# theblackcat102/edgedict

Hardware: NVIDIA H100
Metric: audio-sec/sec E6D2 B=32 T=1000 U=128 V=1024 training step (higher is better)
Workload: dtype bf16

## Files before the change

### edgedict_b200/csrc/elementwise.cu

```cuda
#include "common.cuh"
#include "../../include/edgedict_b200.h"

namespace {

constexpr int LN_WARPS = 8;

template <int PL>
__global__ void __launch_bounds__(LN_WARPS * 32)
layernorm_fwd_kernel(const float* __restrict__ x, const float* __restrict__ res,
                     const float* __restrict__ gamma, const float* __restrict__ beta,
                     float* __restrict__ y, __nv_bfloat16* __restrict__ y16,
                     float* __restrict__ mean, float* __restrict__ rstd, long rows, int H, float eps) {
    const int lane = threadIdx.x & 31;
    const long wstride = (long)gridDim.x * LN_WARPS;
    for (long r = (long)blockIdx.x * LN_WARPS + (threadIdx.x >> 5); r < rows; r += wstride) {
        const float* xr = x + r * H;
        const float* rr = res ? res + r * H : nullptr;
        float v[PL];
        float s = 0.f;
#pragma unroll
        for (int i = 0; i < PL; ++i) {
            int c = lane + i * 32;
            v[i] = 0.f;
            if (c < H) {
                float t = xr[c];
                if (rr) t += rr[c];
                v[i] = t;
                s += t;
            }
        }
        const float mu = warp_sum(s) / H;
        float q = 0.f;
#pragma unroll
        for (int i = 0; i < PL; ++i) {
            int c = lane + i * 32;
            if (c < H) { float d = v[i] - mu; q += d * d; }
        }
        const float rs = rsqrtf(warp_sum(q) / H + eps);
        if (lane == 0) {
            if (mean) mean[r] = mu;
            if (rstd) rstd[r] = rs;
        }
#pragma unroll
        for (int i = 0; i < PL; ++i) {
            int c = lane + i * 32;
            if (c < H) {
                float o = (v[i] - mu) * rs * gamma[c] + beta[c];
                y[r * H + c] = o;
                if (y16) y16[r * H + c] = __float2bfloat16(o);
            }
        }
    }
}

template <int PL>
__global__ void __launch_bounds__(LN_WARPS * 32)
layernorm_bwd_kernel(const float* __restrict__ dy, const float* __restrict__ x,
                     const float* __restrict__ res, const float* __restrict__ gamma,
                     const float* __restrict__ mean, const float* __restrict__ rstd,
                     float* __restrict__ dz, long rows, int H) {
    const int lane = threadIdx.x & 31, w = threadIdx.x >> 5;
    const long wstride = (long)gridDim.x * LN_WARPS;
    for (long r = (long)blockIdx.x * LN_WARPS + w; r < rows; r += wstride) {
        const float mu = mean[r], rs = rstd[r];
        float xh[PL], g[PL];
        float s1 = 0.f, s2 = 0.f;
#pragma unroll
        for (int i = 0; i < PL; ++i) {
            int c = lane + i * 32;
            xh[i] = 0.f; g[i] = 0.f;
            if (c < H) {
                float z = x[r * H + c];
                if (res) z += res[r * H + c];
                xh[i] = (z - mu) * rs;
                g[i] = dy[r * H + c] * gamma[c];
                s1 += g[i];
                s2 += g[i] * xh[i];
            }
        }
        s1 = warp_sum(s1) / H;
        s2 = warp_sum(s2) / H;
#pragma unroll
        for (int i = 0; i < PL; ++i) {
            int c = lane + i * 32;
            if (c < H) dz[r * H + c] = rs * (g[i] - s1 - xh[i] * s2);
        }
    }
}

constexpr int LNB_WARPS = 4;
template <int NV>
__global__ void __launch_bounds__(LNB_WARPS * 32)
layernorm_bwd_fused_kernel(const float* __restrict__ dy, const float* __restrict__ x, const float* __restrict__ res,
                           const float* __restrict__ gamma, const float* __restrict__ mean,
                           const float* __restrict__ rstd, float* __restrict__ dz, long rows, int H) {
    const int lane = threadIdx.x & 31, w = threadIdx.x >> 5;
    const int H4 = H >> 2;
    const long wstride = (long)gridDim.x * LNB_WARPS;
    const float inv_h = 1.f / (float)H;
    const float4* g4 = reinterpret_cast<const float4*>(gamma);
    for (long r = (long)blockIdx.x * LNB_WARPS + w; r < rows; r += wstride) {
        const float mu = mean[r], rs = rstd[r];
        const float4* dy4 = reinterpret_cast<const float4*>(dy + r * H);
        const float4* x4 = reinterpret_cast<const float4*>(x + r * H);
        const float4* r4 = res ? reinterpret_cast<const float4*>(res + r * H) : nullptr;
        float4 d[NV], xh[NV];
        float s1 = 0.f, s2 = 0.f;
#pragma unroll
        for (int i = 0; i < NV; ++i) {
            const int c = lane + i * 32;
            d[i] = make_float4(0.f, 0.f, 0.f, 0.f); xh[i] = d[i];
            if (c < H4) {
                d[i] = dy4[c];
                float4 z = x4[c];
                if (r4) { const float4 q = r4[c]; z.x += q.x; z.y += q.y; z.z += q.z; z.w += q.w; }
                xh[i] = make_float4((z.x - mu) * rs, (z.y - mu) * rs, (z.z - mu) * rs, (z.w - mu) * rs);
                const float4 gm = __ldg(g4 + c);
                const float4 g = make_float4(d[i].x * gm.x, d[i].y * gm.y, d[i].z * gm.z, d[i].w * gm.w);
                s1 += (g.x + g.y) + (g.z + g.w);
                s2 += (g.x * xh[i].x + g.y * xh[i].y) + (g.z * xh[i].z + g.w * xh[i].w);
            }
        }
        s1 = warp_sum(s1) * inv_h;
        s2 = warp_sum(s2) * inv_h;
        float4* dz4 = reinterpret_cast<float4*>(dz + r * H);
#pragma unroll
        for (int i = 0; i < NV; ++i) {
            const int c = lane + i * 32;
            if (c < H4) {
                const float4 gm = __ldg(g4 + c);
                dz4[c] = make_float4(rs * (d[i].x * gm.x - s1 - xh[i].x * s2), rs * (d[i].y * gm.y - s1 - xh[i].y * s2),
                                     rs * (d[i].z * gm.z - s1 - xh[i].z * s2), rs * (d[i].w * gm.w - s1 - xh[i].w * s2));
            }
        }
    }
}

__global__ void __launch_bounds__(1024) layernorm_param_grad_kernel(const float* __restrict__ dy, const float* __restrict__ x,
                                                                     const float* __restrict__ res,
                                                                     const float* __restrict__ mean,
                                                                     const float* __restrict__ rstd, float* __restrict__ dgamma,
                                                                     float* __restrict__ dbeta, long rows, int H) {
    __shared__ float sg[128][9], sb[128][9];
    const int cx = threadIdx.x & 7, k = threadIdx.x >> 3;
    const int c = blockIdx.x * 8 + cx;
    float ag = 0.f, ab = 0.f;
    if (c < H) {
        for (long r = k; r < rows; r += 128) {
            float z = x[r * H + c];
            if (res) z += res[r * H + c];
            const float d = dy[r * H + c];
            ag += d * (z - mean[r]) * rstd[r];
            ab += d;
        }
    }
    sg[k][cx] = ag;
    sb[k][cx] = ab;
    __syncthreads();
#pragma unroll 1
    for (int st = 64; st > 0; st >>= 1) {
        if (k < st) { sg[k][cx] += sg[k + st][cx]; sb[k][cx] += sb[k + st][cx]; }
        __syncthreads();
    }
    if (k == 0 && c < H) {
        dgamma[c] += sg[0][cx];
        dbeta[c] += sb[0][cx];
    }
}

__global__ void time_reduce_fwd_kernel(const float* __restrict__ x, float* __restrict__ y,
                                       __nv_bfloat16* __restrict__ y16, int B, int T, int H) {
    const int T2 = (T + 1) / 2;
    const long n = (long)B * T2 * H;
    for (long i = (long)blockIdx.x * blockDim.x + threadIdx.x; i < n; i += (long)gridDim.x * blockDim.x) {
        int c = (int)(i % H);
        long bt = i / H;
        int t2 = (int)(bt % T2);
        int b = (int)(bt / T2);
        float a = x[((long)b * T + 2 * t2) * H + c];
        float bb = (2 * t2 + 1 < T) ? x[((long)b * T + 2 * t2 + 1) * H + c] : 0.f;
        float o = (a + bb) * 0.5f;
        y[i] = o;
        if (y16) y16[i] = __float2bfloat16(o);
    }
}
__global__ void time_reduce_bwd_kernel(const float* __restrict__ dy, float* __restrict__ dx, int B,
                                       int T, int H) {
    const int T2 = (T + 1) / 2;
    const long n = (long)B * T * H;
    for (long i = (long)blockIdx.x * blockDim.x + threadIdx.x; i < n; i += (long)gridDim.x * blockDim.x) {
        int c = (int)(i % H);
        long bt = i / H;
        int t = (int)(bt % T);
        int b = (int)(bt / T);
        dx[i] = 0.5f * dy[((long)b * T2 + t / 2) * H + c];
    }
}

template <typename I>
__global__ void embedding_fwd_kernel(const I* __restrict__ ids, const float* __restrict__ W,
                                     float* __restrict__ out, __nv_bfloat16* __restrict__ out16,
                                     int B, int U, int E, int prepend, int bos) {
    const int U1 = U + prepend;
    const long n = (long)B * U1 * E;
    for (long i = (long)blockIdx.x * blockDim.x + threadIdx.x; i < n; i += (long)gridDim.x * blockDim.x) {
        int e = (int)(i % E);
        long bu = i / E;
        int u = (int)(bu % U1);
        int b = (int)(bu / U1);
        long id = (prepend && u == 0) ? bos : (long)ids[(long)b * U + u - prepend];
        float v = W[id * E + e];
        out[i] = v;
        if (out16) out16[i] = __float2bfloat16(v);
    }
}
template <typename I>
__device__ __forceinline__ long emb_id(const I* ids, long pos, int U, int U1, int prepend, int bos) {
    const long b = pos / U1;
    const int u = (int)(pos % U1);
    return (prepend && u == 0) ? bos : (long)ids[b * U + u - prepend];
}
template <typename I>
__global__ void embedding_bwd_kernel(const I* __restrict__ ids, const float* __restrict__ dout,
                                     float* __restrict__ dW, int B, int U, int E, int prepend,
                                     int bos, int pad) {
    const int U1 = U + prepend;
    const long n = (long)B * U1;
    const int lane = threadIdx.x & 31;
    for (long i = ((long)blockIdx.x * blockDim.x + threadIdx.x) >> 5; i < n; i += ((long)gridDim.x * blockDim.x) >> 5) {
        const long id = emb_id(ids, i, U, U1, prepend, bos);
        if (id == pad) continue;
        bool first = true;
        for (long j = lane; j < i && first; j += 32) first = emb_id(ids, j, U, U1, prepend, bos) != id;
        if (!__all_sync(0xffffffffu, first)) continue;
        for (int e = lane; e < E; e += 32) {
            float acc = 0.f;
            for (long j = i; j < n; ++j)
                if (emb_id(ids, j, U, U1, prepend, bos) == id) acc += dout[j * E + e];
            dW[id * E + e] += acc;
        }
    }
}

__device__ __forceinline__ float tanh_fast(float x) {
    float y;
    asm("tanh.approx.f32 %0, %1;" : "=f"(y) : "f"(x));
    return y;
}
__device__ __forceinline__ uint32_t pack_bf16(float a, float b) {
    __nv_bfloat162 v = __floats2bfloat162_rn(a, b);
    return *reinterpret_cast<uint32_t*>(&v);
}
__device__ __forceinline__ float2 unpack_bf16(uint32_t u) {
    return __bfloat1622float2(*reinterpret_cast<__nv_bfloat162*>(&u));
}

__global__ void joint_hidden_fwd_f32_kernel(const float* __restrict__ ep, const float* __restrict__ dp,
                                            float* __restrict__ hid, int T, int U, int J) {
    const long bt = blockIdx.x;
    const int b = (int)(bt / T);
    const float* e = ep + bt * J;
    const float* d = dp + (long)b * U * J;
    float* o = hid + bt * (long)U * J;
    for (int i = threadIdx.x; i < U * J; i += blockDim.x) o[i] = tanhf(e[i % J] + d[i]);
}

__global__ void joint_hidden_fwd_bf16_kernel(const float* __restrict__ ep, const float* __restrict__ dp,
                                             __nv_bfloat16* __restrict__ hid, int T, int U, int J) {
    const long bt = blockIdx.x;
    const int b = (int)(bt / T);
    const int J8 = J / 8;
    for (int q = threadIdx.x; q < J8; q += blockDim.x) {
        const float4 e0 = *reinterpret_cast<const float4*>(ep + bt * J + q * 8);
        const float4 e1 = *reinterpret_cast<const float4*>(ep + bt * J + q * 8 + 4);
        const float* d = dp + (long)b * U * J + q * 8;
        __nv_bfloat16* o = hid + bt * (long)U * J + q * 8;
#pragma unroll 4
        for (int u = 0; u < U; ++u) {
            const float4 d0 = *reinterpret_cast<const float4*>(d + (long)u * J);
            const float4 d1 = *reinterpret_cast<const float4*>(d + (long)u * J + 4);
            uint4 v;
            v.x = pack_bf16(tanh_fast(e0.x + d0.x), tanh_fast(e0.y + d0.y));
            v.y = pack_bf16(tanh_fast(e0.z + d0.z), tanh_fast(e0.w + d0.w));
            v.z = pack_bf16(tanh_fast(e1.x + d1.x), tanh_fast(e1.y + d1.y));
            v.w = pack_bf16(tanh_fast(e1.z + d1.z), tanh_fast(e1.w + d1.w));
            *reinterpret_cast<uint4*>(o + (long)u * J) = v;
        }
    }
}

__global__ void joint_hidden_bwd_t_f32_kernel(float* __restrict__ dh, const float* __restrict__ hid,
                                              float* __restrict__ dep, int T, int U, int J) {
    const long bt = blockIdx.x;
    float* g = dh + bt * (long)U * J;
    const float* h = hid + bt * (long)U * J;
    for (int j = threadIdx.x; j < J; j += blockDim.x) {
        float acc = 0.f;
        for (int u = 0; u < U; ++u) {
            float hv = h[(long)u * J + j];
            float pv = g[(long)u * J + j] * (1.f - hv * hv);
            g[(long)u * J + j] = pv;
            acc += pv;
        }
        dep[bt * J + j] = acc;
    }
}
__global__ void joint_hidden_bwd_t_bf16_kernel(__nv_bfloat16* __restrict__ dh, const __nv_bfloat16* __restrict__ hid,
                                               float* __restrict__ dep, int T, int U, int J) {
    const long bt = blockIdx.x;
    const int J8 = J / 8;
    for (int q = threadIdx.x; q < J8; q += blockDim.x) {
        __nv_bfloat16* g = dh + bt * (long)U * J + q * 8;
        const __nv_bfloat16* h = hid + bt * (long)U * J + q * 8;
        float acc[8] = {0.f, 0.f, 0.f, 0.f, 0.f, 0.f, 0.f, 0.f};
#pragma unroll 4
        for (int u = 0; u < U; ++u) {
            const uint4 hv = *reinterpret_cast<const uint4*>(h + (long)u * J);
            uint4 gv = *reinterpret_cast<const uint4*>(g + (long)u * J);
            const uint32_t hw[4] = {hv.x, hv.y, hv.z, hv.w};
            uint32_t gw[4] = {gv.x, gv.y, gv.z, gv.w};
#pragma unroll
            for (int i = 0; i < 4; ++i) {
                const float2 hf = unpack_bf16(hw[i]), gf = unpack_bf16(gw[i]);
                const float p0 = gf.x * (1.f - hf.x * hf.x), p1 = gf.y * (1.f - hf.y * hf.y);
                acc[2 * i] += p0;
                acc[2 * i + 1] += p1;
                gw[i] = pack_bf16(p0, p1);
            }
            *reinterpret_cast<uint4*>(g + (long)u * J) = make_uint4(gw[0], gw[1], gw[2], gw[3]);
        }
        float* o = dep + bt * J + q * 8;
        *reinterpret_cast<float4*>(o) = make_float4(acc[0], acc[1], acc[2], acc[3]);
        *reinterpret_cast<float4*>(o + 4) = make_float4(acc[4], acc[5], acc[6], acc[7]);
    }
}
__global__ void joint_dep_reduce_bf16_kernel(const __nv_bfloat16* __restrict__ dpre, float* __restrict__ dep, int U, int J) {
    const long bt = blockIdx.x;
    const int J8 = J / 8;
    for (int q = threadIdx.x; q < J8; q += blockDim.x) {
        const __nv_bfloat16* g = dpre + bt * (long)U * J + q * 8;
        float acc[8] = {0.f, 0.f, 0.f, 0.f, 0.f, 0.f, 0.f, 0.f};
#pragma unroll 8
        for (int u = 0; u < U; ++u) {
            const uint4 gv = *reinterpret_cast<const uint4*>(g + (long)u * J);
            const uint32_t gw[4] = {gv.x, gv.y, gv.z, gv.w};
#pragma unroll
            for (int i = 0; i < 4; ++i) {
                const float2 gf = unpack_bf16(gw[i]);
                acc[2 * i] += gf.x;
                acc[2 * i + 1] += gf.y;
            }
        }
        float* o = dep + bt * J + q * 8;
        *reinterpret_cast<float4*>(o) = make_float4(acc[0], acc[1], acc[2], acc[3]);
        *reinterpret_cast<float4*>(o + 4) = make_float4(acc[4], acc[5], acc[6], acc[7]);
    }
}
__global__ void joint_hidden_bwd_u_f32_kernel(const float* __restrict__ dpre, float* __restrict__ ddp, int T,
                                              int U, int J) {
    const int b = blockIdx.x / U, u = blockIdx.x % U;
    const float* g = dpre + ((long)b * T * U + u) * J;
    for (int j = threadIdx.x; j < J; j += blockDim.x) {
        float acc = 0.f;
        for (int t = 0; t < T; ++t) acc += g[(long)t * U * J + j];
        ddp[((long)b * U + u) * J + j] = acc;
    }
}
__global__ void joint_hidden_bwd_u_bf16_kernel(const __nv_bfloat16* __restrict__ dpre, float* __restrict__ ddp,
                                               int T, int U, int J) {
    const int b = blockIdx.x / U, u = blockIdx.x % U;
    const int t0 = 0, t1 = T;
    const int J8 = J / 8;
    for (int q = threadIdx.x; q < J8; q += blockDim.x) {
        const __nv_bfloat16* g = dpre + ((long)b * T * U + u) * J + q * 8;
        float acc[8] = {0.f, 0.f, 0.f, 0.f, 0.f, 0.f, 0.f, 0.f};
#pragma unroll 4
        for (int t = t0; t < t1; ++t) {
            const uint4 gv = *reinterpret_cast<const uint4*>(g + (long)t * U * J);
            const uint32_t gw[4] = {gv.x, gv.y, gv.z, gv.w};
#pragma unroll
            for (int i = 0; i < 4; ++i) {
                const float2 gf = unpack_bf16(gw[i]);
                acc[2 * i] += gf.x;
                acc[2 * i + 1] += gf.y;
            }
        }
        float* o = ddp + ((long)b * U + u) * J + q * 8;
        *reinterpret_cast<float4*>(o) = make_float4(acc[0], acc[1], acc[2], acc[3]);
        *reinterpret_cast<float4*>(o + 4) = make_float4(acc[4], acc[5], acc[6], acc[7]);
    }
}

template <int RL, int CW>
__device__ __forceinline__ float colsum_tree(float (*sh)[CW + 1], float v, int k, int cx) {
    sh[k][cx] = v;
    __syncthreads();
#pragma unroll 1
    for (int st = RL / 2; st > 0; st >>= 1) {
        if (k < st) sh[k][cx] += sh[k + st][cx];
        __syncthreads();
    }
    return sh[0][cx];
}
template <typename TI>
__global__ void __launch_bounds__(1024) colsum_kernel(const TI* __restrict__ x, float* __restrict__ out, long rows, int N) {
    __shared__ float sh[32][33];
    const int cx = threadIdx.x & 31, k = threadIdx.x >> 5;
    const int c = blockIdx.x * 32 + cx;
    float acc = 0.f;
    if (c < N)
        for (long r = k; r < rows; r += 32) acc += (float)x[r * N + c];
    const float t = colsum_tree<32, 32>(sh, acc, k, cx);
    if (k == 0 && c < N) out[c] += t;
}

__global__ void __launch_bounds__(1024) colsum_bf16_vec_kernel(const __nv_bfloat16* __restrict__ x, float* __restrict__ out,
                                                               long rows, int N) {
    __shared__ float sh[512][17];
    const int half = threadIdx.x & 1, k = threadIdx.x >> 1;
    const int c0 = blockIdx.x * 16 + half * 8;
    float acc[8] = {0.f, 0.f, 0.f, 0.f, 0.f, 0.f, 0.f, 0.f};
    if (c0 < N) {
        const __nv_bfloat16* p = x + (long)k * N + c0;
        const long step = 512L * N;
        long r = k;
        for (; r + 3 * 512 < rows; r += 4 * 512) {
            uint4 v[4];
#pragma unroll
            for (int q = 0; q < 4; ++q) v[q] = *reinterpret_cast<const uint4*>(p + q * step);
#pragma unroll
            for (int q = 0; q < 4; ++q) {
                const uint32_t w[4] = {v[q].x, v[q].y, v[q].z, v[q].w};
#pragma unroll
                for (int i = 0; i < 4; ++i) {
                    const float2 f = __bfloat1622float2(*reinterpret_cast<const __nv_bfloat162*>(&w[i]));
                    acc[2 * i] += f.x;
                    acc[2 * i + 1] += f.y;
                }
            }
            p += 4 * step;
        }
        for (; r < rows; r += 512, p += step) {
            const uint4 v = *reinterpret_cast<const uint4*>(p);
            const uint32_t w[4] = {v.x, v.y, v.z, v.w};
#pragma unroll
            for (int i = 0; i < 4; ++i) {
                const float2 f = __bfloat1622float2(*reinterpret_cast<const __nv_bfloat162*>(&w[i]));
                acc[2 * i] += f.x;
                acc[2 * i + 1] += f.y;
            }
        }
    }
#pragma unroll 1
    for (int i = 0; i < 8; ++i) {
        const float t = colsum_tree<512, 16>(sh, acc[i], k, half * 8 + i);
        if (k == 0 && c0 < N) out[c0 + i] += t;
        __syncthreads();
    }
}

__global__ void cast_bf16_kernel(const float* __restrict__ x, __nv_bfloat16* __restrict__ y, long n) {
    long i = ((long)blockIdx.x * blockDim.x + threadIdx.x) * 4;
    const long stride = (long)gridDim.x * blockDim.x * 4;
    for (; i + 3 < n; i += stride) {
        float4 v = *reinterpret_cast<const float4*>(x + i);
        __nv_bfloat162 a = __floats2bfloat162_rn(v.x, v.y), b = __floats2bfloat162_rn(v.z, v.w);
        uint2 q;
        q.x = *reinterpret_cast<uint32_t*>(&a);
        q.y = *reinterpret_cast<uint32_t*>(&b);
        *reinterpret_cast<uint2*>(y + i) = q;
    }
    if (i < n) for (long k = i; k < n && k < i + 4; ++k) y[k] = __float2bfloat16(x[k]);
}

template <typename TI>
__global__ void transpose_to_bf16_kernel(const TI* __restrict__ x, __nv_bfloat16* __restrict__ y,
                                         long rows, long cols) {
    __shared__ float tile[32][33];
    long c0 = (long)blockIdx.x * 32, r0 = (long)blockIdx.y * 32;
    for (int i = threadIdx.y; i < 32; i += blockDim.y) {
        long r = r0 + i, c = c0 + threadIdx.x;
        tile[i][threadIdx.x] = (r < rows && c < cols) ? (float)x[r * cols + c] : 0.f;
    }
    __syncthreads();
    for (int i = threadIdx.y; i < 32; i += blockDim.y) {
        long c = c0 + i, r = r0 + threadIdx.x;
        if (r < rows && c < cols) y[c * rows + r] = __float2bfloat16(tile[threadIdx.x][i]);
    }
}

__global__ void adam_kernel(float* __restrict__ p, const float* __restrict__ g, float* __restrict__ m,
                            float* __restrict__ v, long n, float lr, float b1, float b2, float eps,
                            float wd, float bc1, float bc2, float gscale) {
    for (long i = (long)blockIdx.x * blockDim.x + threadIdx.x; i < n; i += (long)gridDim.x * blockDim.x) {
        float gi = g[i] * gscale;
        if (wd != 0.f) gi += wd * p[i];
        float mi = b1 * m[i] + (1.f - b1) * gi;
        float vi = b2 * v[i] + (1.f - b2) * gi * gi;
        m[i] = mi;
        v[i] = vi;
        float denom = sqrtf(vi) / sqrtf(bc2) + eps;
        p[i] -= (lr / bc1) * (mi / denom);
    }
}

__global__ void adam_ex_kernel(float* __restrict__ p, const float* __restrict__ g, float* __restrict__ m,
                               float* __restrict__ v, long n, float lr, float b1, float b2, float eps, float wd,
                               float bc1, float bc2, float gscale, const float* __restrict__ sumsq, float max_norm,
                               int adamw) {
    float coef = gscale;
    if (sumsq) {
        const float norm = sqrtf(*sumsq) * fabsf(gscale);
        if (!isfinite(norm)) return;
        if (max_norm > 0.f) {
            const float c = max_norm / (norm + 1e-6f);
            if (c < 1.f) coef *= c;
        }
    }
    for (long i = (long)blockIdx.x * blockDim.x + threadIdx.x; i < n; i += (long)gridDim.x * blockDim.x) {
        float gi = g[i] * coef;
        const float pi = p[i];
        if (!adamw && wd != 0.f) gi += wd * pi;
        const float mi = b1 * m[i] + (1.f - b1) * gi;
        const float vi = b2 * v[i] + (1.f - b2) * gi * gi;
        m[i] = mi;
        v[i] = vi;
        if (adamw) p[i] = pi - (lr * sqrtf(bc2) / bc1) * (wd * pi + mi / (sqrtf(vi) + eps));
        else p[i] = pi - (lr / bc1) * (mi / (sqrtf(vi) / sqrtf(bc2) + eps));
    }
}

__global__ void sumsq_kernel(const float* __restrict__ x, long n, float* __restrict__ out) {
    __shared__ float sh[33];
    float acc = 0.f;
    for (long i = (long)blockIdx.x * blockDim.x + threadIdx.x; i < n; i += (long)gridDim.x * blockDim.x)
        acc += x[i] * x[i];
    acc = block_sum(acc, sh);
    if (threadIdx.x == 0) atomicAdd(out, acc);
}

inline int ew_grid(long n, int threads) {
    long b = (n + threads - 1) / threads;
    long cap = (long)eb_num_sms() * 32;
    return (int)(b < 1 ? 1 : (b < cap ? b : cap));
}

}

#define ST(s) reinterpret_cast<cudaStream_t>(s)

EB_API int eb_layernorm_fwd(const float* x, const float* res, const float* gamma, const float* beta,
                            float* y, void* y_bf16, float* mean, float* rstd, long rows, int H,
                            float eps, void* stream) {
    if (!x || !gamma || !beta || !y || rows <= 0 || H <= 0 || H > 2048) return EB_ERR_INVALID;
    long blocks = (rows + LN_WARPS - 1) / LN_WARPS;
    long cap = (long)eb_num_sms() * 8;
    int grid = (int)(blocks < cap ? blocks : cap);
#define LN_FWD(PL) layernorm_fwd_kernel<PL><<<grid, LN_WARPS * 32, 0, ST(stream)>>>( \
        x, res, gamma, beta, y, (__nv_bfloat16*)y_bf16, mean, rstd, rows, H, eps)
    if (H <= 256) LN_FWD(8); else if (H <= 512) LN_FWD(16); else if (H <= 1024) LN_FWD(32); else LN_FWD(64);
#undef LN_FWD
    EB_CHECK_LAUNCH();
    return EB_OK;
}

EB_API int eb_layernorm_bwd(const float* dy, const float* x, const float* res, const float* gamma,
                            const float* mean, const float* rstd, float* dz, float* dgamma,
                            float* dbeta, long rows, int H, void* stream) {
    if (!dy || !x || !gamma || !mean || !rstd || !dz || !dgamma || !dbeta || H > 2048)
        return EB_ERR_INVALID;
    const bool vec_ok = H % 128 == 0 && H <= 1024 && rows > 0 &&
                        ((reinterpret_cast<uintptr_t>(dy) | reinterpret_cast<uintptr_t>(x) | reinterpret_cast<uintptr_t>(dz) |
                          reinterpret_cast<uintptr_t>(gamma) | (res ? reinterpret_cast<uintptr_t>(res) : 0)) & 15) == 0;
    if (vec_ok) {
        long blocks_f = (rows + LNB_WARPS - 1) / LNB_WARPS;
        long cap_f = (long)eb_num_sms() * 3;
        const int grid_f = (int)(blocks_f < cap_f ? blocks_f : cap_f);
#define LN_BWDF(NV) layernorm_bwd_fused_kernel<NV><<<grid_f, LNB_WARPS * 32, 0, ST(stream)>>>( \
        dy, x, res, gamma, mean, rstd, dz, rows, H)
        if (H <= 128) LN_BWDF(1); else if (H <= 256) LN_BWDF(2); else if (H <= 512) LN_BWDF(4); else LN_BWDF(8);
#undef LN_BWDF
    } else {
        long blocks = (rows + LN_WARPS - 1) / LN_WARPS;
        long cap = (long)eb_num_sms() * 8;
        int grid = (int)(blocks < cap ? blocks : cap);
#define LN_BWD(PL) layernorm_bwd_kernel<PL><<<grid, LN_WARPS * 32, 0, ST(stream)>>>( \
        dy, x, res, gamma, mean, rstd, dz, rows, H)
        if (H <= 256) LN_BWD(8); else if (H <= 512) LN_BWD(16); else if (H <= 1024) LN_BWD(32); else LN_BWD(64);
#undef LN_BWD
    }
    EB_CHECK_LAUNCH();
    layernorm_param_grad_kernel<<<(H + 7) / 8, 1024, 0, ST(stream)>>>(dy, x, res, mean, rstd, dgamma, dbeta, rows, H);
    EB_CHECK_LAUNCH();
    return EB_OK;
}

EB_API int eb_time_reduce_fwd(const float* x, float* y, void* y_bf16, int B, int T, int H, void* stream) {
    long n = (long)B * ((T + 1) / 2) * H;
    time_reduce_fwd_kernel<<<ew_grid(n, 256), 256, 0, ST(stream)>>>(x, y, (__nv_bfloat16*)y_bf16, B, T, H);
    EB_CHECK_LAUNCH();
    return EB_OK;
}
EB_API int eb_time_reduce_bwd(const float* dy, float* dx, int B, int T, int H, void* stream) {
    long n = (long)B * T * H;
    time_reduce_bwd_kernel<<<ew_grid(n, 256), 256, 0, ST(stream)>>>(dy, dx, B, T, H);
    EB_CHECK_LAUNCH();
    return EB_OK;
}

EB_API int eb_embedding_fwd(const void* ids, int ids_are_int64, const float* W, float* out,
                            void* out_bf16, int B, int U, int E, int prepend_bos, int bos, void* stream) {
    long n = (long)B * (U + (prepend_bos ? 1 : 0)) * E;
    if (n <= 0) return EB_OK;
    if (ids_are_int64)
        embedding_fwd_kernel<long long><<<ew_grid(n, 256), 256, 0, ST(stream)>>>(
            (const long long*)ids, W, out, (__nv_bfloat16*)out_bf16, B, U, E, prepend_bos ? 1 : 0, bos);
    else
        embedding_fwd_kernel<int><<<ew_grid(n, 256), 256, 0, ST(stream)>>>(
            (const int*)ids, W, out, (__nv_bfloat16*)out_bf16, B, U, E, prepend_bos ? 1 : 0, bos);
    EB_CHECK_LAUNCH();
    return EB_OK;
}
EB_API int eb_embedding_bwd(const void* ids, int ids_are_int64, const float* dout, float* dW, int B,
                            int U, int E, int prepend_bos, int bos, int pad, void* stream) {
    const long npos = (long)B * (U + (prepend_bos ? 1 : 0));
    if (npos <= 0 || E <= 0) return EB_OK;
    const long n = npos * 32;
    if (ids_are_int64)
        embedding_bwd_kernel<long long><<<ew_grid(n, 256), 256, 0, ST(stream)>>>(
            (const long long*)ids, dout, dW, B, U, E, prepend_bos ? 1 : 0, bos, pad);
    else
        embedding_bwd_kernel<int><<<ew_grid(n, 256), 256, 0, ST(stream)>>>(
            (const int*)ids, dout, dW, B, U, E, prepend_bos ? 1 : 0, bos, pad);
    EB_CHECK_LAUNCH();
    return EB_OK;
}

EB_API int eb_joint_hidden_fwd(const float* ep, const float* dp, void* hidden, int hidden_bf16, int B,
                               int T, int U, int J, void* stream) {
    if (!ep || !dp || !hidden) return EB_ERR_INVALID;
    if (hidden_bf16) {
        if (J % 8) return EB_ERR_INVALID;
        joint_hidden_fwd_bf16_kernel<<<B * T, 96, 0, ST(stream)>>>(ep, dp, (__nv_bfloat16*)hidden, T, U, J);
    } else {
        joint_hidden_fwd_f32_kernel<<<B * T, 256, 0, ST(stream)>>>(ep, dp, (float*)hidden, T, U, J);
    }
    EB_CHECK_LAUNCH();
    return EB_OK;
}

EB_API int eb_joint_hidden_bwd(void* dhidden_inout, const void* hidden, int is_bf16, float* dep,
                               float* ddp, int B, int T, int U, int J, void* stream) {
    if (!dhidden_inout || !hidden || !dep || !ddp) return EB_ERR_INVALID;
    if (is_bf16) {
        if (J % 8) return EB_ERR_INVALID;
        joint_hidden_bwd_t_bf16_kernel<<<B * T, 96, 0, ST(stream)>>>(
            (__nv_bfloat16*)dhidden_inout, (const __nv_bfloat16*)hidden, dep, T, U, J);
        EB_CHECK_LAUNCH();
        joint_hidden_bwd_u_bf16_kernel<<<B * U, 96, 0, ST(stream)>>>((const __nv_bfloat16*)dhidden_inout, ddp, T, U, J);
    } else {
        joint_hidden_bwd_t_f32_kernel<<<B * T, 256, 0, ST(stream)>>>(
            (float*)dhidden_inout, (const float*)hidden, dep, T, U, J);
        EB_CHECK_LAUNCH();
        joint_hidden_bwd_u_f32_kernel<<<B * U, 256, 0, ST(stream)>>>((const float*)dhidden_inout, ddp, T, U, J);
    }
    EB_CHECK_LAUNCH();
    return EB_OK;
}

EB_API int eb_joint_dpre_reduce(const void* dpre16, float* dep, float* ddp, int B, int T, int U, int J, void* stream) {
    if (!dpre16 || !dep || !ddp || B <= 0 || T <= 0 || U <= 0 || J <= 0 || J % 8 ||
        (reinterpret_cast<uintptr_t>(dpre16) & 15) || (reinterpret_cast<uintptr_t>(dep) & 15))
        return EB_ERR_INVALID;
    joint_dep_reduce_bf16_kernel<<<B * T, 96, 0, ST(stream)>>>((const __nv_bfloat16*)dpre16, dep, U, J);
    EB_CHECK_LAUNCH();
    joint_hidden_bwd_u_bf16_kernel<<<B * U, 96, 0, ST(stream)>>>((const __nv_bfloat16*)dpre16, ddp, T, U, J);
    EB_CHECK_LAUNCH();
    return EB_OK;
}

EB_API int eb_colsum(const void* x, int x_bf16, float* out, long rows, int N, void* stream) {
    if (!x || !out || rows <= 0 || N <= 0) return EB_ERR_INVALID;
    if (x_bf16 && N % 8 == 0 && (reinterpret_cast<uintptr_t>(x) & 15) == 0)
        colsum_bf16_vec_kernel<<<(N + 15) / 16, 1024, 0, ST(stream)>>>((const __nv_bfloat16*)x, out, rows, N);
    else if (x_bf16)
        colsum_kernel<__nv_bfloat16><<<(N + 31) / 32, 1024, 0, ST(stream)>>>((const __nv_bfloat16*)x, out, rows, N);
    else
        colsum_kernel<float><<<(N + 31) / 32, 1024, 0, ST(stream)>>>((const float*)x, out, rows, N);
    EB_CHECK_LAUNCH();
    return EB_OK;
}

EB_API int eb_cast_bf16(const float* x, void* y, long n, void* stream) {
    if (n <= 0) return EB_OK;
    if ((reinterpret_cast<uintptr_t>(x) & 15) || (reinterpret_cast<uintptr_t>(y) & 7)) return EB_ERR_INVALID;
    cast_bf16_kernel<<<ew_grid((n + 3) / 4, 256), 256, 0, ST(stream)>>>(x, (__nv_bfloat16*)y, n);
    EB_CHECK_LAUNCH();
    return EB_OK;
}

EB_API int eb_transpose_to_bf16(const void* x, int x_bf16, void* y, long rows, long cols, void* stream) {
    dim3 grid((unsigned)((cols + 31) / 32), (unsigned)((rows + 31) / 32));
    if (x_bf16)
        transpose_to_bf16_kernel<__nv_bfloat16><<<grid, dim3(32, 8), 0, ST(stream)>>>(
            (const __nv_bfloat16*)x, (__nv_bfloat16*)y, rows, cols);
    else
        transpose_to_bf16_kernel<float><<<grid, dim3(32, 8), 0, ST(stream)>>>((const float*)x, (__nv_bfloat16*)y, rows, cols);
    EB_CHECK_LAUNCH();
    return EB_OK;
}

EB_API int eb_adam_step(float* p, const float* g, float* m, float* v, long n, float lr, float beta1,
                        float beta2, float eps, float weight_decay, int step, float grad_scale,
                        void* stream) {
    if (!p || !g || !m || !v || n <= 0 || step < 1) return EB_ERR_INVALID;
    float bc1 = 1.f - powf(beta1, (float)step), bc2 = 1.f - powf(beta2, (float)step);
    adam_kernel<<<ew_grid(n, 256), 256, 0, ST(stream)>>>(p, g, m, v, n, lr, beta1, beta2, eps,
                                                         weight_decay, bc1, bc2, grad_scale);
    EB_CHECK_LAUNCH();
    return EB_OK;
}

EB_API int eb_adam_step_ex(float* p, const float* g, float* m, float* v, long n, float lr, float beta1, float beta2,
                           float eps, float weight_decay, int step, float grad_scale, const float* sumsq,
                           float max_norm, int adamw, void* stream) {
    if (!p || !g || !m || !v || n <= 0 || step < 1) return EB_ERR_INVALID;
    float bc1 = 1.f - powf(beta1, (float)step), bc2 = 1.f - powf(beta2, (float)step);
    adam_ex_kernel<<<ew_grid(n, 256), 256, 0, ST(stream)>>>(p, g, m, v, n, lr, beta1, beta2, eps, weight_decay, bc1, bc2,
                                                            grad_scale, sumsq, max_norm, adamw);
    EB_CHECK_LAUNCH();
    return EB_OK;
}

EB_API int eb_sumsq(const float* x, long n, float* out_accum, void* stream) {
    sumsq_kernel<<<ew_grid(n, 256), 256, 0, ST(stream)>>>(x, n, out_accum);
    EB_CHECK_LAUNCH();
    return EB_OK;
}
```

### edgedict_b200/csrc/gemm_tc.cu

```cuda
#include <cuda.h>
#include <stdlib.h>
#include "common.cuh"
#include "sm90.cuh"
#include "../../include/edgedict_b200.h"

namespace {

constexpr int BM = 128, BK = 64, UMMA_K = 16;
constexpr int A_BYTES = BM * BK * 2;
constexpr int NTHREADS = 2 * 128 + 32;
template <int BN_, bool LOW_ = false> struct Cfg {
    static constexpr int STAGES = LOW_ ? 3 : (BN_ == 256 ? 4 : 6);
    static constexpr int B_BYTES = BN_ * BK * 2;
    static constexpr int STAGE_BYTES = A_BYTES + B_BYTES;
    static constexpr int SMEM_BYTES = 1024 + STAGES * STAGE_BYTES + 256;
};

struct Sched {
    long num_m; int num_n; int ksplit; long out_tiles; bool n_inner;
    unsigned wid, nw;
    __device__ __forceinline__ bool get(long j, long& m_blk, int& n_blk, int& ks) const {
        if (n_inner) {
            const long grp = (long)wid + (j / num_n) * nw;
            if (grp >= num_m) return false;
            m_blk = grp; n_blk = (int)(j % num_n); ks = 0;
            return true;
        }
        const long wi = (long)wid + j * nw;
        if (wi >= out_tiles * ksplit) return false;
        const long tile = wi % out_tiles;
        ks = (int)(wi / out_tiles);
        m_blk = tile / num_n; n_blk = (int)(tile % num_n);
        return true;
    }
};

struct LseArgs {
    const int* labels; const int* xlen; const int* ylen;
    float* denom; float* lpb; float* lpl;
    int maxT, maxU, blank;
    const __nv_bfloat16* aux;
};

__device__ __forceinline__ void st_bf16x2(__nv_bfloat16* p, float a, float b) {
    *reinterpret_cast<__nv_bfloat162*>(p) = __floats2bfloat162_rn(a, b);
}

template <bool A_MN, bool B_MN, int BN_, bool LSE = false, bool LOW_ = false>
__global__ void __launch_bounds__(NTHREADS, LOW_ ? 2 : 1)
gemm_tc_kernel(const __grid_constant__ CUtensorMap tma_a, const __grid_constant__ CUtensorMap tma_b,
               void* __restrict__ Cout, int c_bf16, const float* __restrict__ bias, int accumulate,
               long M, int N, long K, int ksplit, LseArgs lse = LseArgs(), float* __restrict__ part = nullptr) {
    using C_ = Cfg<BN_, LOW_>;
    constexpr int BN = BN_, STAGES = C_::STAGES, STAGE_BYTES = C_::STAGE_BYTES, NACC = BN / 2;
    extern __shared__ uint8_t smem_raw[];
    uint8_t* smem = reinterpret_cast<uint8_t*>((reinterpret_cast<uintptr_t>(smem_raw) + 1023) & ~uintptr_t(1023));
    uint8_t* tiles = smem;
    uint64_t* bars = reinterpret_cast<uint64_t*>(smem + STAGES * STAGE_BYTES);
    const uint32_t full0 = smem_u32(bars), empty0 = smem_u32(bars + STAGES);

    const int warp = threadIdx.x >> 5, lane = threadIdx.x & 31;
    const long num_m = (M + BM - 1) / BM;
    const int num_n = (N + BN - 1) / BN;
    Sched sch;
    sch.num_m = num_m; sch.num_n = num_n; sch.ksplit = ksplit; sch.out_tiles = num_m * num_n;
    sch.wid = blockIdx.x; sch.nw = gridDim.x;
    sch.n_inner = LSE || ((ksplit == 1) && (num_m >= 2L * sch.nw));
    const int nkb_total = (int)((K + BK - 1) / BK);
    const int kb_per = (nkb_total + ksplit - 1) / ksplit;

    if (threadIdx.x == 0) {
        for (int s = 0; s < STAGES; ++s) { mbar_init(full0 + 8 * s, 1); mbar_init(empty0 + 8 * s, 8); }
        asm volatile("fence.mbarrier_init.release.cluster;" ::: "memory");
        asm volatile("prefetch.tensormap [%0];" :: "l"(&tma_a) : "memory");
        asm volatile("prefetch.tensormap [%0];" :: "l"(&tma_b) : "memory");
    }
    __syncthreads();

    if (warp == 8) {
        if (lane == 0) {
            int stage = 0; uint32_t phase = 0;
            long mb; int nb, ksx;
            constexpr uint32_t TX = A_BYTES + C_::B_BYTES;
            for (long jj = 0; sch.get(jj, mb, nb, ksx); ++jj) {
                const int kb0 = ksx * kb_per, kb1 = min(nkb_total, kb0 + kb_per);
                const int m0 = (int)mb * BM, n0 = nb * BN;
                for (int kb = kb0; kb < kb1; ++kb) {
                    mbar_wait(empty0 + 8 * stage, phase ^ 1);
                    const uint32_t sa = smem_u32(tiles + stage * STAGE_BYTES), sb = sa + A_BYTES;
                    const uint32_t fb = full0 + 8 * stage;
                    mbar_expect_tx(fb, TX);
                    if (!A_MN) tma_load_2d(sa, &tma_a, kb * BK, m0, fb);
                    else { tma_load_2d(sa, &tma_a, m0, kb * BK, fb); tma_load_2d(sa + 8192, &tma_a, m0 + 64, kb * BK, fb); }
                    if (!B_MN) tma_load_2d(sb, &tma_b, kb * BK, n0, fb);
                    else {
#pragma unroll
                        for (int bx = 0; bx < BN / 64; ++bx) tma_load_2d(sb + bx * 8192, &tma_b, n0 + bx * 64, kb * BK, fb);
                    }
                    if (++stage == STAGES) { stage = 0; phase ^= 1; }
                }
            }
        }
        return;
    }

    const int wg = warp >> 2;
    const int r_in = 64 * wg + 16 * (warp & 3) + (lane >> 2);
    const int cq = 2 * (lane & 3);
    float* Cf = reinterpret_cast<float*>(Cout);
    __nv_bfloat16* const Ch = reinterpret_cast<__nv_bfloat16*>(Cout);
    const bool vec2 = (N % 2) == 0;
    float acc[NACC];
    int stage = 0; uint32_t phase = 0;
    long mb; int nb, ks;
    float rm[2] = {-INFINITY, -INFINITY}, rs[2] = {0.f, 0.f}, xb[2] = {0.f, 0.f}, xl[2] = {0.f, 0.f};
    int lab[2] = {-1, -1};
    bool cell_ok[2] = {false, false};
    for (long jj = 0; sch.get(jj, mb, nb, ks); ++jj) {
        const int kb0 = ks * kb_per, kb1 = min(nkb_total, kb0 + kb_per);
        const long m0 = mb * BM;
        const int n0 = nb * BN;
#pragma unroll
        for (int i = 0; i < NACC; ++i) acc[i] = 0.f;
        int prev = -1;
        for (int kb = kb0; kb < kb1; ++kb) {
            mbar_wait(full0 + 8 * stage, phase);
            const uint32_t sa = smem_u32(tiles + stage * STAGE_BYTES) + (uint32_t)wg * 8192u, sb = smem_u32(tiles + stage * STAGE_BYTES) + A_BYTES;
            wgmma_fence();
#pragma unroll
            for (int k = 0; k < BK / UMMA_K; ++k) {
                const uint64_t ad = A_MN ? make_desc(sa + k * 2048, 8192, 1024) : make_desc(sa + k * 32, 16, 1024);
                const uint64_t bd = B_MN ? make_desc(sb + k * 2048, 8192, 1024) : make_desc(sb + k * 32, 16, 1024);
                if constexpr (BN == 256) wgmma_m64n256k16<A_MN ? 1 : 0, B_MN ? 1 : 0>(acc, ad, bd, 1);
                else wgmma_m64n128k16<A_MN ? 1 : 0, B_MN ? 1 : 0>(acc, ad, bd, 1);
            }
            wgmma_commit();
            wgmma_wait<1>();
            if (prev >= 0 && lane == 0) mbar_arrive(empty0 + 8 * prev);
            prev = stage;
            if (++stage == STAGES) { stage = 0; phase ^= 1; }
        }
        wgmma_wait<0>();
        wgmma_fence_regs(acc);
        if (prev >= 0 && lane == 0) mbar_arrive(empty0 + 8 * prev);

        if constexpr (LSE) {
            constexpr float LOG2E = 1.4426950408889634f;
            if (nb == 0) {
#pragma unroll
                for (int h = 0; h < 2; ++h) {
                    rm[h] = -INFINITY; rs[h] = 0.f; xb[h] = 0.f; xl[h] = 0.f; lab[h] = -1; cell_ok[h] = false;
                    const long cell = m0 + r_in + 8 * h;
                    if (cell < M) {
                        const int u = (int)(cell % lse.maxU);
                        const long bt = cell / lse.maxU;
                        const int t = (int)(bt % lse.maxT), b = (int)(bt / lse.maxT);
                        const int Tn = lse.xlen[b], Un = lse.ylen[b] + 1;
                        cell_ok[h] = t < Tn && u < Un;
                        if (cell_ok[h] && u < Un - 1) lab[h] = lse.labels[b * (lse.maxU - 1) + u];
                    }
                }
            }
#pragma unroll
            for (int h = 0; h < 2; ++h) {
                float cm = -INFINITY;
#pragma unroll
                for (int i = 0; i < BN / 8; ++i) {
                    const int col = n0 + 8 * i + cq;
                    float v0 = acc[4 * i + 2 * h], v1 = acc[4 * i + 2 * h + 1];
                    v0 = col < N ? v0 + (bias ? __ldg(bias + col) : 0.f) : -INFINITY;
                    v1 = col + 1 < N ? v1 + (bias ? __ldg(bias + col + 1) : 0.f) : -INFINITY;
                    acc[4 * i + 2 * h] = v0; acc[4 * i + 2 * h + 1] = v1;
                    cm = fmaxf(cm, fmaxf(v0, v1));
                    if (col == lse.blank) xb[h] = v0;
                    if (col + 1 == lse.blank) xb[h] = v1;
                    if (col == lab[h]) xl[h] = v0;
                    if (col + 1 == lab[h]) xl[h] = v1;
                }
                const float nm = fmaxf(rm[h], cm);
                if (nm != -INFINITY) {
                    const float nml = nm * LOG2E;
                    float a0 = 0.f, a1 = 0.f;
#pragma unroll
                    for (int i = 0; i < BN / 8; ++i) {
                        a0 += fast_ex2(fmaf(acc[4 * i + 2 * h], LOG2E, -nml));
                        a1 += fast_ex2(fmaf(acc[4 * i + 2 * h + 1], LOG2E, -nml));
                    }
                    rs[h] = rs[h] * fast_ex2((rm[h] - nm) * LOG2E) + (a0 + a1);
                    rm[h] = nm;
                }
                const long row = m0 + r_in + 8 * h;
                if (row < M) {
#pragma unroll
                    for (int i = 0; i < BN / 8; ++i) {
                        const int col = n0 + 8 * i + cq;
                        __nv_bfloat16* cp = Ch + row * N + col;
                        if (vec2 && col + 1 < N) st_bf16x2(cp, acc[4 * i + 2 * h], acc[4 * i + 2 * h + 1]);
                        else {
                            if (col < N) cp[0] = __float2bfloat16(acc[4 * i + 2 * h]);
                            if (col + 1 < N) cp[1] = __float2bfloat16(acc[4 * i + 2 * h + 1]);
                        }
                    }
                }
            }
            if (nb == num_n - 1) {
#pragma unroll
                for (int h = 0; h < 2; ++h) {
#pragma unroll
                    for (int o = 1; o <= 2; o <<= 1) {
                        const float m2 = __shfl_xor_sync(0xffffffffu, rm[h], o), s2 = __shfl_xor_sync(0xffffffffu, rs[h], o);
                        xb[h] += __shfl_xor_sync(0xffffffffu, xb[h], o);
                        xl[h] += __shfl_xor_sync(0xffffffffu, xl[h], o);
                        const float m = fmaxf(rm[h], m2);
                        rs[h] = (rm[h] == -INFINITY ? 0.f : rs[h] * fast_ex2((rm[h] - m) * LOG2E)) +
                                (m2 == -INFINITY ? 0.f : s2 * fast_ex2((m2 - m) * LOG2E));
                        rm[h] = m;
                    }
                    if ((lane & 3) == 0 && cell_ok[h]) {
                        const long cell = m0 + r_in + 8 * h;
                        const float d = -(rm[h] + logf(rs[h]));
                        lse.denom[cell] = d;
                        lse.lpb[cell] = d + xb[h];
                        lse.lpl[cell] = d + xl[h];
                    }
                }
            }
        } else {
            const bool add_bias = bias && ks == 0;
            if (ksplit > 1) Cf = part + (long)ks * M * N;
            const int acc_c = ksplit > 1 ? 0 : accumulate;
#pragma unroll
            for (int h = 0; h < 2; ++h) {
                const long row = m0 + r_in + 8 * h;
                if (row >= M) continue;
#pragma unroll
                for (int i = 0; i < BN / 8; ++i) {
                    const int col = n0 + 8 * i + cq;
                    if (col >= N) break;
                    const bool two = col + 1 < N, pair = two && vec2;
                    float v0 = acc[4 * i + 2 * h], v1 = acc[4 * i + 2 * h + 1];
                    if (add_bias) { v0 += __ldg(bias + col); if (two) v1 += __ldg(bias + col + 1); }
                    const long off = row * N + col;
                    if (c_bf16) {
                        __nv_bfloat16* cp = Ch + off;
                        if (lse.aux) {
                            float h0, h1 = 0.f;
                            if (pair) {
                                const float2 hh = __bfloat1622float2(__ldg(reinterpret_cast<const __nv_bfloat162*>(lse.aux + off)));
                                h0 = hh.x; h1 = hh.y;
                            } else {
                                h0 = __bfloat162float(lse.aux[off]);
                                if (two) h1 = __bfloat162float(lse.aux[off + 1]);
                            }
                            v0 *= 1.f - h0 * h0; v1 *= 1.f - h1 * h1;
                        }
                        if (pair) {
                            if (accumulate) {
                                const float2 o = __bfloat1622float2(*reinterpret_cast<const __nv_bfloat162*>(cp));
                                v0 += o.x; v1 += o.y;
                            }
                            st_bf16x2(cp, v0, v1);
                        } else {
                            if (accumulate) { v0 += __bfloat162float(cp[0]); if (two) v1 += __bfloat162float(cp[1]); }
                            cp[0] = __float2bfloat16(v0);
                            if (two) cp[1] = __float2bfloat16(v1);
                        }
                    } else {
                        float* cp = Cf + off;
                        if (pair) {
                            if (acc_c) { const float2 o = *reinterpret_cast<const float2*>(cp); v0 += o.x; v1 += o.y; }
                            *reinterpret_cast<float2*>(cp) = make_float2(v0, v1);
                        } else {
                            if (acc_c) { v0 += cp[0]; if (two) v1 += cp[1]; }
                            cp[0] = v0;
                            if (two) cp[1] = v1;
                        }
                    }
                }
            }
        }
    }
}

__global__ void splitk_reduce_kernel(const float* __restrict__ part, int ksplit, long mn, float* __restrict__ C, int accumulate) {
    for (long i = (long)blockIdx.x * blockDim.x + threadIdx.x; i < mn; i += (long)gridDim.x * blockDim.x) {
        float v = accumulate ? C[i] : 0.f;
        for (int s = 0; s < ksplit; ++s) v += part[(long)s * mn + i];
        C[i] = v;
    }
}

int choose_ksplit(long out_tiles, long nkb, long workers, double r) {
    int ksplit = 1;
    long cap = nkb / 16;
    if (cap > 64) cap = 64;
    double best = -1.0;
    for (long ks = 1; ks <= cap; ++ks) {
        const long items = out_tiles * ks;
        const long waves = (items + workers - 1) / workers;
        const double score = (double)items / (double)(waves * workers) / (1.0 + r * (double)ks / (double)nkb);
        if (score > best) { best = score; ksplit = (int)ks; }
    }
    return ksplit;
}

template <bool A_MN, bool B_MN, int BN_, bool LSE, bool LOW_>
int launch_kernel(const CUtensorMap& ta, const CUtensorMap& tb, void* C, int c_bf16, const float* bias, int accumulate,
                  long M, int N, long K, int ksplit, long work, const LseArgs& ea, cudaStream_t st, float* part = nullptr) {
    using C_ = Cfg<BN_, LOW_>;
    auto kern = gemm_tc_kernel<A_MN, B_MN, BN_, LSE, LOW_>;
    static bool attr_done = false;
    if (!attr_done) {
        EB_CUDA(cudaFuncSetAttribute(kern, cudaFuncAttributeMaxDynamicSharedMemorySize, C_::SMEM_BYTES));
        attr_done = true;
    }
    const int grid = (int)(work < eb_num_sms() ? work : eb_num_sms());
    kern<<<grid, NTHREADS, C_::SMEM_BYTES, st>>>(ta, tb, C, c_bf16, bias, accumulate, M, N, K, ksplit, ea, part);
    EB_CHECK_LAUNCH();
    if (ksplit > 1) {
        const long mn = M * (long)N;
        const long blocks = (mn + 255) / 256, cap = 4L * eb_num_sms();
        splitk_reduce_kernel<<<(int)(blocks < cap ? blocks : cap), 256, 0, st>>>(part, ksplit, mn, (float*)C, accumulate);
        EB_CHECK_LAUNCH();
    }
    return EB_OK;
}

template <bool A_MN, bool B_MN, int BN_>
int launch(const CUtensorMap& ta, const CUtensorMap& tb, void* C, int c_bf16, const float* bias, int accumulate,
           long M, int N, long K, int ksplit, float* part, cudaStream_t st, const void* aux = nullptr) {
    LseArgs ea = LseArgs();
    ea.aux = reinterpret_cast<const __nv_bfloat16*>(aux);
    const long out_tiles = ((M + BM - 1) / BM) * ((N + BN_ - 1) / BN_);
    return launch_kernel<A_MN, B_MN, BN_, false, false>(ta, tb, C, c_bf16, bias, accumulate, M, N, K, ksplit,
                                                        out_tiles * ksplit, ea, st, part);
}

void plan(int a_mn_major, int c_bf16, int accumulate, long M, int N, long K, int flags, bool& wide, int& ksplit) {
    const bool low = (flags & EB_GEMM_CORESIDENT) != 0;
    static int force_bn = -1;
    if (force_bn < 0) { const char* e = getenv("EDGEDICT_GEMM_BN"); force_bn = e ? atoi(e) : 0; }
    const long wide_tiles = ((M + BM - 1) / BM) * (N / 256);
    wide = (N % 256 == 0) && (wide_tiles >= eb_num_sms() || (!c_bf16 && (K + BK - 1) / BK >= 64 && wide_tiles >= 8));
    if (!wide && N % 256 == 128 && N >= 512 && (M + BM - 1) / BM >= 4L * eb_num_sms() && accumulate == 0) wide = true;
    if (force_bn == 128) wide = false;
    if (force_bn == 256 && N % 128 == 0) wide = true;
    if (low) wide = false;
    (void)a_mn_major;
    const int BN = wide ? 256 : 128;
    const long out_tiles = ((M + BM - 1) / BM) * ((N + BN - 1) / BN);
    const long nkb = (K + BK - 1) / BK;
    ksplit = 1;
    if (!low && !c_bf16 && nkb >= 64 && out_tiles < eb_num_sms())
        ksplit = choose_ksplit(out_tiles, nkb, eb_num_sms(), BN == 256 ? 32.0 : 16.0);
}

int launch_low(const CUtensorMap& ta, const CUtensorMap& tb, void* C, int c_bf16, const float* bias, int accumulate,
               long M, int N, long K, cudaStream_t st) {
    const long tiles = ((M + BM - 1) / BM) * ((N + 127) / 128);
    return launch_kernel<false, false, 128, false, true>(ta, tb, C, c_bf16, bias, accumulate, M, N, K, 1, tiles, LseArgs(), st);
}

int launch_lse(const CUtensorMap& ta, const CUtensorMap& tb, void* C, const float* bias, long M, int N, long K,
               const LseArgs& lse, cudaStream_t st) {
    return launch_kernel<false, false, 128, true, false>(ta, tb, C, 1, bias, 0, M, N, K, 1, (M + BM - 1) / BM, lse, st);
}

}

EB_API int eb_joint_logits_lse(const void* hidden16, const void* w2_16, const float* b2, void* logits16,
                               const int* labels, const int* xlen, const int* ylen, float* denom, float* lpb,
                               float* lpl, int B, int maxT, int maxU, int V, int J, int blank, void* stream) {
    if (!hidden16 || !w2_16 || !logits16 || !xlen || !ylen || !denom || !lpb || !lpl || (!labels && maxU > 1) ||
        B <= 0 || maxT <= 0 || maxU <= 0 || V <= 0 || J <= 0 || J % 8 || blank < 0 || blank >= V)
        return EB_ERR_INVALID;
    if ((reinterpret_cast<uintptr_t>(hidden16) & 15) || (reinterpret_cast<uintptr_t>(w2_16) & 15) ||
        (b2 && (reinterpret_cast<uintptr_t>(b2) & 15)))
        return EB_ERR_INVALID;
    const long M = (long)B * maxT * maxU;
    CUtensorMap ta, tb;
    if (!make_map(&ta, hidden16, (uint64_t)J, (uint64_t)M, 128) || !make_map(&tb, w2_16, (uint64_t)J, (uint64_t)V, 128)) {
        fprintf(stderr, "[edgedict_b200] cuTensorMapEncodeTiled failed\n");
        return EB_ERR_CUDA;
    }
    LseArgs lse;
    lse.labels = labels; lse.xlen = xlen; lse.ylen = ylen; lse.denom = denom; lse.lpb = lpb; lse.lpl = lpl;
    lse.maxT = maxT; lse.maxU = maxU; lse.blank = blank; lse.aux = nullptr;
    cudaStream_t st = reinterpret_cast<cudaStream_t>(stream);
    return launch_lse(ta, tb, logits16, b2, M, V, J, lse, st);
}

EB_API int eb_gemm_bf16(const void* A, int a_mn_major, const void* B, int b_mn_major, void* C, int c_bf16,
                        const float* bias, int accumulate, long M, int N, long K, void* stream) {
    return eb_gemm_bf16_ex(A, a_mn_major, B, b_mn_major, C, c_bf16, bias, accumulate, M, N, K, 0, nullptr, 0, stream);
}

static int gemm_dispatch(const void* A, int a_mn_major, const void* B, int b_mn_major, void* C, int c_bf16,
                         const float* bias, int accumulate, long M, int N, long K, int flags, const void* aux,
                         float* partials, long partial_floats, void* stream);

EB_API long eb_gemm_bf16_partials(int a_mn_major, int c_bf16, int accumulate, long M, int N, long K, int flags) {
    if (M <= 0 || N <= 0 || K <= 0) return 0;
    bool wide;
    int ksplit;
    plan(a_mn_major, c_bf16, accumulate, M, N, K, flags, wide, ksplit);
    return ksplit > 1 ? (long)ksplit * M * N : 0;
}

EB_API int eb_gemm_bf16_ex(const void* A, int a_mn_major, const void* B, int b_mn_major, void* C, int c_bf16,
                           const float* bias, int accumulate, long M, int N, long K, int flags, float* partials,
                           long partial_floats, void* stream) {
    return gemm_dispatch(A, a_mn_major, B, b_mn_major, C, c_bf16, bias, accumulate, M, N, K, flags, nullptr, partials,
                         partial_floats, stream);
}

EB_API int eb_gemm_bf16_dtanh(const void* A, int a_mn_major, const void* B, int b_mn_major, void* C16,
                              const void* hid16, long M, int N, long K, void* stream) {
    if (!hid16 || (reinterpret_cast<uintptr_t>(hid16) & 7) || (reinterpret_cast<uintptr_t>(C16) & 7) || N % 4) return EB_ERR_INVALID;
    return gemm_dispatch(A, a_mn_major, B, b_mn_major, C16, 1, nullptr, 0, M, N, K, 0, hid16, nullptr, 0, stream);
}

static int gemm_dispatch(const void* A, int a_mn_major, const void* B, int b_mn_major, void* C, int c_bf16,
                         const float* bias, int accumulate, long M, int N, long K, int flags, const void* aux,
                         float* partials, long partial_floats, void* stream) {
    if (!A || !B || !C || M <= 0 || N <= 0 || K <= 0) return EB_ERR_INVALID;
    const bool low = (flags & EB_GEMM_CORESIDENT) != 0;
    if (low && (a_mn_major || b_mn_major)) return EB_ERR_INVALID;
    if ((reinterpret_cast<uintptr_t>(A) & 15) || (reinterpret_cast<uintptr_t>(B) & 15)) return EB_ERR_INVALID;
    if ((a_mn_major ? M : K) % 8 || (b_mn_major ? (long)N : K) % 8) return EB_ERR_INVALID;
    bool wide;
    int ksplit;
    plan(a_mn_major, c_bf16, accumulate, M, N, K, flags, wide, ksplit);
    if (ksplit > 1) {
        const long fit = (partials && (reinterpret_cast<uintptr_t>(partials) & 7) == 0) ? partial_floats / (M * (long)N) : 0;
        if (fit < ksplit) ksplit = fit > 1 ? (int)fit : 1;
    }
    CUtensorMap ta, tb;
    bool ok = a_mn_major ? make_map(&ta, A, (uint64_t)M, (uint64_t)K, 64) : make_map(&ta, A, (uint64_t)K, (uint64_t)M, 128);
    ok = ok && (b_mn_major ? make_map(&tb, B, (uint64_t)N, (uint64_t)K, 64)
                           : make_map(&tb, B, (uint64_t)K, (uint64_t)N, wide ? 256 : 128));
    if (!ok) {
        fprintf(stderr, "[edgedict_b200] cuTensorMapEncodeTiled failed\n");
        return EB_ERR_CUDA;
    }
    cudaStream_t st = reinterpret_cast<cudaStream_t>(stream);
    if (low) return launch_low(ta, tb, C, c_bf16, bias, accumulate, M, N, K, st);
#define EB_GO(AM, BMN)                                                                                          \
    return wide ? launch<AM, BMN, 256>(ta, tb, C, c_bf16, bias, accumulate, M, N, K, ksplit, partials, st, aux) \
                : launch<AM, BMN, 128>(ta, tb, C, c_bf16, bias, accumulate, M, N, K, ksplit, partials, st, aux)
    if (a_mn_major) {
        if (b_mn_major) { EB_GO(true, true); }
        EB_GO(true, false);
    }
    if (b_mn_major) { EB_GO(false, true); }
    EB_GO(false, false);
#undef EB_GO
}
```

Measured before the change: 10730.

## Split bf16 colsum across 4-CTA cluster and prefetch tanh aux in GEMM epilogue

The bf16 column-sum kernel now runs as a 4-CTA thread-block cluster, each CTA covering a quarter of the row lanes with a deeper 8-way unrolled load loop. Partial sums are combined through distributed shared memory before a single tree reduction in rank 0, which raises parallelism for narrow N. In the GEMM dtanh epilogue, the aux (hidden) values for a whole row are preloaded into registers before the store loop, and aux GEMMs are forced to use the 128-wide tile. This adds cluster syncs and register pressure, and it may lose the efficiency of wide tiles for those GEMMs.

```diff
diff --git a/edgedict_b200/csrc/elementwise.cu b/edgedict_b200/csrc/elementwise.cu
--- a/edgedict_b200/csrc/elementwise.cu
+++ b/edgedict_b200/csrc/elementwise.cu
@@ -1,5 +1,8 @@
+#include <cooperative_groups.h>
 #include "common.cuh"
 #include "../../include/edgedict_b200.h"
+
+namespace cg = cooperative_groups;
 
 namespace {
 
@@ -414,22 +417,25 @@
     if (k == 0 && c < N) out[c] += t;
 }
 
-__global__ void __launch_bounds__(1024) colsum_bf16_vec_kernel(const __nv_bfloat16* __restrict__ x, float* __restrict__ out,
-                                                               long rows, int N) {
-    __shared__ float sh[512][17];
-    const int half = threadIdx.x & 1, k = threadIdx.x >> 1;
+constexpr int COLSUM_LANES = 512, COLSUM_CL = 4, COLSUM_CTA_LANES = COLSUM_LANES / COLSUM_CL;
+__global__ void __cluster_dims__(1, COLSUM_CL, 1) __launch_bounds__(2 * COLSUM_CTA_LANES)
+colsum_bf16_vec_kernel(const __nv_bfloat16* __restrict__ x, float* __restrict__ out, long rows, int N) {
+    __shared__ float sh[COLSUM_CTA_LANES][17];
+    cg::cluster_group cluster = cg::this_cluster();
+    const unsigned rank = cluster.block_rank();
+    const int half = threadIdx.x & 1, kl = threadIdx.x >> 1, k = (int)rank * COLSUM_CTA_LANES + kl;
     const int c0 = blockIdx.x * 16 + half * 8;
     float acc[8] = {0.f, 0.f, 0.f, 0.f, 0.f, 0.f, 0.f, 0.f};
     if (c0 < N) {
         const __nv_bfloat16* p = x + (long)k * N + c0;
-        const long step = 512L * N;
+        const long step = (long)COLSUM_LANES * N;
         long r = k;
-        for (; r + 3 * 512 < rows; r += 4 * 512) {
-            uint4 v[4];
-#pragma unroll
-            for (int q = 0; q < 4; ++q) v[q] = *reinterpret_cast<const uint4*>(p + q * step);
-#pragma unroll
-            for (int q = 0; q < 4; ++q) {
+        for (; r + 7 * COLSUM_LANES < rows; r += 8 * COLSUM_LANES) {
+            uint4 v[8];
+#pragma unroll
+            for (int q = 0; q < 8; ++q) v[q] = *reinterpret_cast<const uint4*>(p + q * step);
+#pragma unroll
+            for (int q = 0; q < 8; ++q) {
                 const uint32_t w[4] = {v[q].x, v[q].y, v[q].z, v[q].w};
 #pragma unroll
                 for (int i = 0; i < 4; ++i) {
@@ -438,9 +444,9 @@
                     acc[2 * i + 1] += f.y;
                 }
             }
-            p += 4 * step;
-        }
-        for (; r < rows; r += 512, p += step) {
+            p += 8 * step;
+        }
+        for (; r < rows; r += COLSUM_LANES, p += step) {
             const uint4 v = *reinterpret_cast<const uint4*>(p);
             const uint32_t w[4] = {v.x, v.y, v.z, v.w};
 #pragma unroll
@@ -451,12 +457,26 @@
             }
         }
     }
+#pragma unroll
+    for (int i = 0; i < 8; ++i) sh[kl][half * 8 + i] = acc[i];
+    cluster.sync();
+    if (rank < 2) {
+        const float* peer = cluster.map_shared_rank(&sh[0][0], rank + 2);
+        for (int e = threadIdx.x; e < COLSUM_CTA_LANES * 16; e += blockDim.x) sh[e >> 4][e & 15] += peer[(e >> 4) * 17 + (e & 15)];
+    }
+    cluster.sync();
+    if (rank == 0) {
+        const float* peer = cluster.map_shared_rank(&sh[0][0], 1);
+        for (int e = threadIdx.x; e < COLSUM_CTA_LANES * 16; e += blockDim.x) sh[e >> 4][e & 15] += peer[(e >> 4) * 17 + (e & 15)];
+    }
+    cluster.sync();
+    if (rank != 0) return;
 #pragma unroll 1
-    for (int i = 0; i < 8; ++i) {
-        const float t = colsum_tree<512, 16>(sh, acc[i], k, half * 8 + i);
-        if (k == 0 && c0 < N) out[c0 + i] += t;
+    for (int st = COLSUM_CTA_LANES / 2; st > 0; st >>= 1) {
+        for (int e = threadIdx.x; e < st * 16; e += blockDim.x) sh[e >> 4][e & 15] += sh[(e >> 4) + st][e & 15];
         __syncthreads();
     }
+    if (threadIdx.x < 16 && blockIdx.x * 16 + (int)threadIdx.x < N) out[blockIdx.x * 16 + threadIdx.x] += sh[0][threadIdx.x];
 }
 
 __global__ void cast_bf16_kernel(const float* __restrict__ x, __nv_bfloat16* __restrict__ y, long n) {
@@ -682,7 +702,7 @@
 EB_API int eb_colsum(const void* x, int x_bf16, float* out, long rows, int N, void* stream) {
     if (!x || !out || rows <= 0 || N <= 0) return EB_ERR_INVALID;
     if (x_bf16 && N % 8 == 0 && (reinterpret_cast<uintptr_t>(x) & 15) == 0)
-        colsum_bf16_vec_kernel<<<(N + 15) / 16, 1024, 0, ST(stream)>>>((const __nv_bfloat16*)x, out, rows, N);
+        colsum_bf16_vec_kernel<<<dim3((N + 15) / 16, COLSUM_CL), 2 * COLSUM_CTA_LANES, 0, ST(stream)>>>((const __nv_bfloat16*)x, out, rows, N);
     else if (x_bf16)
         colsum_kernel<__nv_bfloat16><<<(N + 31) / 32, 1024, 0, ST(stream)>>>((const __nv_bfloat16*)x, out, rows, N);
     else
diff --git a/edgedict_b200/csrc/gemm_tc.cu b/edgedict_b200/csrc/gemm_tc.cu
--- a/edgedict_b200/csrc/gemm_tc.cu
+++ b/edgedict_b200/csrc/gemm_tc.cu
@@ -233,6 +233,23 @@
             for (int h = 0; h < 2; ++h) {
                 const long row = m0 + r_in + 8 * h;
                 if (row >= M) continue;
+                constexpr bool PRE = BN == 128 && !LOW_;
+                __nv_bfloat162 hx[PRE ? BN / 8 : 1];
+                if constexpr (PRE) {
+                    if (c_bf16 && lse.aux) {
+#pragma unroll
+                        for (int i = 0; i < BN / 8; ++i) {
+                            const int col = n0 + 8 * i + cq;
+                            const long off = row * N + col;
+                            hx[i] = __floats2bfloat162_rn(0.f, 0.f);
+                            if (col + 1 < N && vec2) hx[i] = __ldg(reinterpret_cast<const __nv_bfloat162*>(lse.aux + off));
+                            else if (col < N) {
+                                hx[i].x = lse.aux[off];
+                                if (col + 1 < N) hx[i].y = lse.aux[off + 1];
+                            }
+                        }
+                    }
+                }
 #pragma unroll
                 for (int i = 0; i < BN / 8; ++i) {
                     const int col = n0 + 8 * i + cq;
@@ -245,7 +262,11 @@
                         __nv_bfloat16* cp = Ch + off;
                         if (lse.aux) {
                             float h0, h1 = 0.f;
-                            if (pair) {
+                            if constexpr (PRE) {
+                                const float2 hh = __bfloat1622float2(hx[i]);
+                                h0 = hh.x;
+                                if (two) h1 = hh.y;
+                            } else if (pair) {
                                 const float2 hh = __bfloat1622float2(__ldg(reinterpret_cast<const __nv_bfloat162*>(lse.aux + off)));
                                 h0 = hh.x; h1 = hh.y;
                             } else {
@@ -431,6 +452,7 @@
     bool wide;
     int ksplit;
     plan(a_mn_major, c_bf16, accumulate, M, N, K, flags, wide, ksplit);
+    if (aux) wide = false;
     if (ksplit > 1) {
         const long fit = (partials && (reinterpret_cast<uintptr_t>(partials) & 7) == 0) ? partial_floats / (M * (long)N) : 0;
         if (fit < ksplit) ksplit = fit > 1 ? (int)fit : 1;
```

Result: faster. 11080, median of 6 (+3.2%).
